# nubot-nudt/RDMNet

Measured on AMD Instinct MI355X. Metric: scan-pairs/sec (whole node), higher is better.
Workload: dtype f32

## Files before the change

include/rdmnet_hip.h:

```cpp
#ifndef RDMNET_HIP_H_
#define RDMNET_HIP_H_

#include <stddef.h>
#include <stdint.h>

#ifdef __cplusplus
extern "C" {
#endif

#define RDM_ABI_VERSION 2

int rdm_abi_version(void);
size_t rdm_abi_struct_size(int which);
const char* rdm_last_error(void);

int rdm_rehash_schedule(int64_t max_elems, int64_t* at_host, int64_t* buckets_host, int cap);

size_t rdm_grid_subsample_workspace_bytes(int64_t n_points, int batch);
int rdm_grid_subsample(const float* points, int64_t n_points, const int64_t* lengths, int batch,
                       float voxel_size, float* out_points, int64_t* out_lengths, void* ws,
                       size_t ws_bytes, void* stream);
int rdm_grid_subsample_form(const float* points, int64_t n_points, const int64_t* lengths, int batch, float voxel_size,
                            float* out_points, int64_t* out_lengths, void* ws, size_t ws_bytes, void* stream, int form);

// ... 95 lines not shown
                                  double* out);
size_t rdm_pose_graph_consistency_workspace_bytes(int64_t n_graphs, const int64_t* graph_node_offsets_host,
                                                  const int64_t* graph_edge_offsets_host, const int64_t* edges_host,
                                                  const int64_t* graph_pair_offsets_host, const int64_t* pairs_host);
int rdm_pose_graph_consistency(int64_t n_graphs, const int64_t* graph_node_offsets_host, const int64_t* graph_edge_offsets_host,
                               const double* nodes, const int64_t* edges_host, const double* transforms, const double* informations,
                               const double* weights, const int64_t* graph_pair_offsets_host, const int64_t* pairs_host,
                               const double* pair_transforms, const double* pair_informations, double* covariances_out,
                               double* cross_out, double* residual_cov_out, double* d2_out, uint8_t* pair_status_out,
                               double* report_host, void* ws, size_t ws_bytes, void* stream);
int rdm_pose_graph_pair_covariances_host(int64_t n_nodes, int64_t n_edges, const int64_t* edges_host, const double* diag,
                                         const double* off, int64_t n_pairs, const int64_t* pairs_host, double* out);
int rdm_pose_graph_pair_terms_host(const double* source_pose, const double* target_pose, const double* transform,
                                   const double* information, const double* cov_ss, const double* cov_tt, const double* cov_st,
                                   double* out);
int rdm_dbg_pose_graph_marginals_ticks(long long* device_ticks);

size_t rdm_gemm_workspace_bytes(int64_t m, int64_t n, int batches);
int rdm_gemm(const float* a, int64_t lda, int64_t stride_a, const float* b, int64_t ldb,
             int64_t stride_b, int trans_b, float* c, int64_t ldc, int64_t stride_c, int64_t m,
             int64_t n, int64_t k, int batches, const float* bias, const float* rowdiv, int act,
             void* ws, size_t ws_bytes, void* stream);
int rdm_gemm_last_plan(int* out4_host);

int rdm_kpconv_gather(const float* q_points, int64_t m, const float* s_points, int64_t n_s,
                      const float* s_feats, int64_t c, int64_t ldf, const uint8_t* s_positive,
                      const int64_t* idx, int64_t h, int64_t ldi, const int32_t* width,
                      const float* kernel_points, float sigma, float* wf, int64_t ldw, float* nn,
                      void* stream);
int rdm_kpconv_fused_enabled(void);
int rdm_kpconv_fused_supported(int64_t c_in, int64_t c_out);
int64_t rdm_kpconv_fused_partial_rows(int64_t m, int64_t c_in);
size_t rdm_kpconv_packed_floats(int64_t c_in, int64_t c_out);
int rdm_kpconv_pack_weights(const float* w_host, int64_t c_in, int64_t c_out, float* packed_host);
int rdm_kpconv_fused(const float* q_points, int64_t m, const float* s_points, int64_t n_s, const float* s_feats,
                     int64_t c, int64_t ldf, const uint8_t* s_positive, const int64_t* idx, int64_t h, int64_t ldi,
                     const int32_t* width, const float* kernel_points, float sigma, const float* w_packed,
                     const float* bias, int64_t c_out, float* out, int64_t ldo, double* gn_partial,
                     const float* order_records, void* stream);
int rdm_kpconv_fused_form(const float* q_points, int64_t m, const float* s_points, int64_t n_s, const float* s_feats,
                          int64_t c, int64_t ldf, const uint8_t* s_positive, const int64_t* idx, int64_t h, int64_t ldi,
                          const int32_t* width, const float* kernel_points, float sigma, const float* w_packed,
                          const float* bias, int64_t c_out, float* out, int64_t ldo, double* gn_partial,
                          const float* order_records, int form, void* stream);
size_t rdm_kpconv_fused_workspace_bytes(int64_t m, int64_t c_in, int64_t c_out);
int rdm_kpconv_fused_group_norm(const float* q_points, int64_t m, const float* s_points, int64_t n_s,
// ... 418 lines not shown
```

rdmnet_amd/_lib.py:

```python
import ctypes
import os

_HERE = os.path.dirname(os.path.abspath(__file__))
LIB_PATH = os.environ.get('RDM_LIB_PATH') or os.path.join(_HERE, 'librdmnet_hip.so')

c_void = ctypes.c_void_p
c_i64 = ctypes.c_int64
c_int = ctypes.c_int
c_f32 = ctypes.c_float
c_size = ctypes.c_size_t

ABI_VERSION = 2


class FineMatchingOptions(ctypes.Structure):
    _fields_ = [('topk', ctypes.c_int32), ('mutual', ctypes.c_int32), ('use_dustbin', ctypes.c_int32),
                ('use_global_score', ctypes.c_int32), ('confidence_threshold', ctypes.c_float),
                ('correspondence_limit', ctypes.c_int32)]

    @classmethod
    def of(cls, topk=1, mutual=False, use_dustbin=True, confidence_threshold=0.0, use_global_score=False,
           correspondence_limit=None):
        return cls(int(topk), int(bool(mutual)), int(bool(use_dustbin)), int(bool(use_global_score)), float(confidence_threshold),
                   0 if correspondence_limit is None else int(correspondence_limit))
# ... 36 lines not shown
               'bad_indices')

SIGNATURES = {
    'rdm_abi_version': (c_int, []),
    'rdm_abi_struct_size': (c_size, [c_int]),
    'rdm_last_error': (ctypes.c_char_p, []),
    'rdm_rehash_schedule': (c_int, [c_i64, c_void, c_void, c_int]),
    'rdm_grid_subsample_workspace_bytes': (c_size, [c_i64, c_int]),
    'rdm_grid_subsample': (c_int, [c_void, c_i64, c_void, c_int, c_f32, c_void, c_void, c_void, c_size,
                                   c_void]),
    'rdm_grid_subsample_form': (c_int, [c_void, c_i64, c_void, c_int, c_f32, c_void, c_void, c_void, c_size,
                                        c_void, c_int]),
    'rdm_radius_neighbors_workspace_bytes': (c_size, [c_i64, c_i64, c_int]),
    'rdm_radius_neighbors': (c_int, [c_void, c_i64, c_void, c_i64, c_void, c_void, c_int, c_f32, c_int,
                                     c_void, c_void, c_void, c_void, c_void, c_size, c_void]),
    'rdm_radius_grid_workspace_bytes': (c_size, [c_i64]),
    'rdm_radius_grid_build': (c_int, [c_void, c_i64, c_void, c_int, c_f32, c_void, c_size, c_void]),
    'rdm_radius_grid_query': (c_int, [c_void, c_size, c_i64, c_void, c_i64, c_void, c_int, c_f32, c_int, c_void, c_void,
                                      c_void, c_void, c_void, c_size, c_void]),
    'rdm_gemm_workspace_bytes': (c_size, [c_i64, c_i64, c_int]),
    'rdm_gemm': (c_int, [c_void, c_i64, c_i64, c_void, c_i64, c_i64, c_int, c_void, c_i64, c_i64, c_i64, c_i64,
                         c_i64, c_int, c_void, c_void, c_int, c_void, c_size, c_void]),
    'rdm_gemm_last_plan': (c_int, [c_void]),
    'rdm_kpconv_gather': (c_int, [c_void, c_i64, c_void, c_i64, c_void, c_i64, c_i64, c_void, c_void, c_i64,
                                  c_i64, c_void, c_void, c_f32, c_void, c_i64, c_void, c_void]),
    'rdm_kpconv_gather_ordered': (c_int, [c_void, c_i64, c_void, c_i64, c_void, c_i64, c_i64, c_void, c_void, c_i64,
                                          c_i64, c_void, c_void, c_f32, c_void, c_i64, c_void, c_void, c_void]),
    'rdm_kpconv_gather_form': (c_int, [c_void, c_i64, c_void, c_i64, c_void, c_i64, c_i64, c_void, c_void, c_i64,
                                       c_i64, c_void, c_void, c_f32, c_void, c_i64, c_void, c_void, c_int, c_void]),
    'rdm_kpconv_fused_enabled': (c_int, []),
    'rdm_kpconv_fused_supported': (c_int, [c_i64, c_i64]),
    'rdm_kpconv_fused_partial_rows': (c_i64, [c_i64, c_i64]),
    'rdm_kpconv_packed_floats': (c_size, [c_i64, c_i64]),
    'rdm_kpconv_pack_weights': (c_int, [c_void, c_i64, c_i64, c_void]),
    'rdm_kpconv_fused': (c_int, [c_void, c_i64, c_void, c_i64, c_void, c_i64, c_i64, c_void, c_void, c_i64, c_i64, c_void, c_void,
                                 c_f32, c_void, c_void, c_i64, c_void, c_i64, c_void, c_void, c_void]),
    'rdm_kpconv_fused_form': (c_int, [c_void, c_i64, c_void, c_i64, c_void, c_i64, c_i64, c_void, c_void, c_i64, c_i64, c_void, c_void,
                                      c_f32, c_void, c_void, c_i64, c_void, c_i64, c_void, c_void, c_int, c_void]),
    'rdm_kpconv_fused_workspace_bytes': (c_size, [c_i64, c_i64, c_i64]),
    'rdm_kpconv_fused_group_norm': (c_int, [c_void, c_i64, c_void, c_i64, c_void, c_i64, c_i64, c_void, c_void, c_i64, c_i64, c_void,
                                            c_void, c_f32, c_void, c_void, c_i64, c_int, c_void, c_void, c_f32, c_int, c_void, c_i64,
                                            c_void, c_i64, c_void, c_size, c_void, c_void]),
    'rdm_voxel_downsample_workspace_bytes': (c_size, [c_i64]),
    'rdm_voxel_downsample': (c_int, [c_void, c_i64, c_i64, c_int, ctypes.c_double, c_void, c_i64, c_void, c_void, c_void,
                                     c_size, c_void]),
    'rdm_ransac_workspace_bytes': (c_size, [c_int]),
# ... 270 lines not shown
```

rdmnet_amd/csrc/gemm.hip:

```cpp
#include "../../include/rdmnet_hip.h"
#include <cmath>
#include <cstdlib>

#include "common.h"
#include "internal.h"
#include "lockstep.h"

namespace {

using namespace rdm;

typedef float f32x16 __attribute__((ext_vector_type(16)));
typedef float f32x4_t __attribute__((ext_vector_type(4)));

struct GemmArgs {
  const float* A = nullptr;
  const float* B = nullptr;
  float* C = nullptr;
  const float* bias = nullptr;
  const float* rowdiv = nullptr;
  int M = 0, N = 0, K = 0;
  int lda = 0, ldb = 0, ldc = 0;
  long long sa = 0, sb = 0, sc = 0;
  int act = 0;
  int splits = 1;
  float* part = nullptr;
  double* stats = nullptr;
  const float* A2 = nullptr;
  const int64_t* aidx = nullptr;
  int lda2 = 0, ldi = 0, c1 = 0, n_coarse = 0;
  const int64_t* bidx = nullptr;
  int n_b = 0;
  const float* seed = nullptr;
  const int64_t* sidx = nullptr;
  int ld_seed = 0, ldsi = 0, n_seed = 0;
  int xcd_tiles = 0;
#ifdef RDM_GEMM_TIMING
  unsigned long long* clk = nullptr;
#endif
};
#ifdef RDM_GEMM_TIMING
#define GEMM_STAMP(k) do { if (blockIdx.x == 0 && blockIdx.y == 0 && blockIdx.z == 0 && threadIdx.x == 0) g.clk[k] = __builtin_amdgcn_s_memtime(); } while (0)
#else
#define GEMM_STAMP(k) do { } while (0)
#endif

__device__ __forceinline__ float apply_act(float v, int act) {
  if (act == 1) return v > 0.f ? v : 0.f;
  if (act == 2) return v > 0.f ? v : 0.1f * v;
  return v;
}

template <int BM, int BN, int WM, int WN, int BK, bool TRANS_B, int PF, bool CAT = false, bool SEED = false>
__device__ __forceinline__ void gemm_kernel_body(const dim3 blockIdx, const dim3 gridDim, GemmArgs g) {
  (void)blockIdx; (void)gridDim;
  constexpr int TM = BM / WM, TN = BN / WN, FM = TM / 32, FN = TN / 32;
  static_assert(WM * WN == 4 && TM % 32 == 0 && TN % 32 == 0, "bad tile");
  static_assert(!SEED || (!CAT && !TRANS_B), "seeded accumulators: plain operands only");
  constexpr int LDA_S = BM + 1, LDB_S = TRANS_B ? BN + 1 : BN + 4;
  constexpr int CR = BM < 64 ? BM : 64;
  constexpr int LDC_S = BN + 4;
  constexpr int TPR = BN / 4;
  constexpr int RPI = 256 / TPR;
  constexpr int kBytesAB = (2 * BK * LDA_S + 2 * BK * LDB_S) * 4, kBytesC = CR * LDC_S * 4, kBytesStat = RPI * BN * 2 * 8;
  constexpr int kBytes = kBytesAB > kBytesC ? (kBytesAB > kBytesStat ? kBytesAB : kBytesStat) : (kBytesC > kBytesStat ? kBytesC : kBytesStat);
  static_assert((2 * BK * LDA_S * 4) % 16 == 0 && CR % RPI == 0, "tile layout");
  __shared__ __attribute__((aligned(16))) char smem[kBytes];
  float (*As)[BK][LDA_S] = reinterpret_cast<float (*)[BK][LDA_S]>(smem);
  float (*Bs)[BK][LDB_S] = reinterpret_cast<float (*)[BK][LDB_S]>(smem + 2 * BK * LDA_S * 4);
  float (*Cs)[LDC_S] = reinterpret_cast<float (*)[LDC_S]>(smem);
  double (*stat_red)[1][2] = reinterpret_cast<double (*)[1][2]>(smem);

  const int tid = threadIdx.x, lane = tid & 63, wave = tid >> 6;
  const int wm = wave / WN, wn = wave % WN;
  int tile_x = blockIdx.x, tile_y = blockIdx.y;
  if (g.xcd_tiles) {
    const int nblk = gridDim.x * gridDim.y, lin = blockIdx.y * gridDim.x + blockIdx.x;
    const int q = nblk / 8, rr = nblk % 8, xcd = lin % 8, within = lin / 8;
    const int logical = (xcd < rr ? xcd * (q + 1) : rr * (q + 1) + (xcd - rr) * q) + within;
    tile_x = logical % gridDim.x;
    tile_y = logical / gridDim.x;
  }
  const int m0 = tile_y * BM, n0 = tile_x * BN;
  GEMM_STAMP(0);
  const int batch = blockIdx.z / g.splits, split = blockIdx.z % g.splits;
  const float* A = g.A + batch * g.sa;
  const float* B = g.B + batch * g.sb;

  const int ktiles = (g.K + BK - 1) / BK;
  const int per = (ktiles + g.splits - 1) / g.splits;
  const int kt0 = split * per, kt1 = min(ktiles, kt0 + per);

  constexpr int A_N4 = BM * BK / 4;
  constexpr int A_V = (A_N4 + 255) / 256;
// ... 197 lines not shown
          for (int r = 0; r < 16; ++r) {
            const float v = g.seed[max(seed_row[i][r], 0ll) * g.ld_seed + min(col, g.N - 1)];
            acc[i][j][r] = (seed_row[i][r] >= 0 && col < g.N) ? v : 0.f;
          }
        }
    }
    store_tiles(ra0, rb0, 0, kt0);
  }
  lds_barrier();
  GEMM_STAMP(1);
  if (kt0 < kt1) {
    read_half(af_lo, bf_lo, 0, 0);
    if constexpr (PF == 1) {
      for (int kt = kt0; kt < kt1; ++kt) step(ra0, rb0, ra0, rb0, kt, (kt - kt0) & 1);
    } else {
      for (int kt = kt0; kt < kt1; kt += 2) {
        step(ra0, rb0, ra1, rb1, kt, 0);
        if (kt + 1 < kt1) step(ra1, rb1, ra0, rb0, kt + 1, 1);
      }
    }
  }

  GEMM_STAMP(2);
  const bool stats = g.stats != nullptr && !partial;
  const bool has_rd = !partial && g.rowdiv != nullptr;
  const int act = g.act;
  float* C = partial ? g.part + static_cast<long long>(blockIdx.z) * g.M * g.N : g.C + batch * g.sc;
  const int ldc = partial ? g.N : g.ldc;
  const bool vec_ok = (ldc & 3) == 0 && (reinterpret_cast<uintptr_t>(C) & 15) == 0;
  double cs[4] = {0.0, 0.0, 0.0, 0.0}, css[4] = {0.0, 0.0, 0.0, 0.0};
#pragma unroll
  for (int pass = 0; pass < BM / CR; ++pass) {
#pragma unroll
    for (int i = 0; i < FM; ++i) {
      const int rbase = wm * TM + i * 32 - pass * CR;
      if (rbase < 0 || rbase >= CR) continue;
#pragma unroll
      for (int j = 0; j < FN; ++j)
#pragma unroll
        for (int r = 0; r < 16; ++r) Cs[rbase + (r & 3) + 8 * (r >> 2) + 4 * lk][wn * TN + j * 32 + li] = acc[i][j][r];
    }
    lds_barrier();
    GEMM_STAMP(4);
#pragma unroll
    for (int it = 0; it < CR / RPI; ++it) {
      const int lrow = it * RPI + rsub;
      const int row = m0 + pass * CR + lrow;
      if (row < g.M && gcol < g.N) {
        const float4 t = *reinterpret_cast<const float4*>(&Cs[lrow][c4]);
        float v[4] = {t.x, t.y, t.z, t.w};
        if (has_rd) {
          const float rd = rdv[pass * (CR / RPI) + it];
#pragma unroll
          for (int e = 0; e < 4; ++e) v[e] = v[e] / rd;
        }
        if (!partial) {
#pragma unroll
          for (int e = 0; e < 4; ++e) {
            const float u = v[e] + bv[e];
            const float neg = act == 2 ? 0.1f * u : 0.f;
            v[e] = (act != 0 && !(u > 0.f)) ? neg : u;
          }
        }
        float* dst = C + static_cast<long long>(row) * ldc + gcol;
        if (vec_ok && gcol + 3 < g.N) {
          *reinterpret_cast<float4*>(dst) = make_float4(v[0], v[1], v[2], v[3]);
        } else {
#pragma unroll
          for (int e = 0; e < 4; ++e)
            if (gcol + e < g.N) dst[e] = v[e];
        }
        if (stats) {
#pragma unroll
          for (int e = 0; e < 4; ++e) {
            cs[e] += v[e];
            css[e] += static_cast<double>(v[e]) * v[e];
          }
        }
      }
    }
    GEMM_STAMP(5);
    lds_barrier();
  }
  if (stats) {
#pragma unroll
    for (int e = 0; e < 4; ++e) {
      stat_red[rsub * BN + c4 + e][0][0] = cs[e];
      stat_red[rsub * BN + c4 + e][0][1] = css[e];
    }
    lds_barrier();
    for (int cl = tid; cl < BN; cl += 256) {
      const int col = n0 + cl;
      if (col >= g.N) continue;
      double a = 0.0, b = 0.0;
#pragma unroll
      for (int w = 0; w < RPI; ++w) {
        a += stat_red[w * BN + cl][0][0];
        b += stat_red[w * BN + cl][0][1];
      }
      g.stats[(static_cast<long long>(tile_y) * 2 + 0) * g.N + col] = a;
      g.stats[(static_cast<long long>(tile_y) * 2 + 1) * g.N + col] = b;
    }
  }
  GEMM_STAMP(3);
}

__device__ __forceinline__ void gemm_small_body(const dim3 blockIdx, const GemmArgs& g, float (*red)[32][33]) {
  const int tid = threadIdx.x, lane = tid & 63, wave = tid >> 6;
  const int li = lane & 31, lk = lane >> 5;
  const int m0 = blockIdx.y * 32, n0 = blockIdx.x * 32;
  const int kq = g.K / 4;
  const int kbeg = wave * kq;
  const int row = min(m0 + li, g.M - 1);
  const int col = n0 + li;
  const bool col_ok = col < g.ldb;
  const float* arow = g.A + static_cast<long long>(row) * g.lda;
  f32x16 acc;
#pragma unroll
  for (int r = 0; r < 16; ++r) acc[r] = 0.f;
  for (int c = 0; c < kq; c += 32) {
    float a[16], b[16];
    const int kb = kbeg + c + lk * 16;
#pragma unroll
    for (int q = 0; q < 4; ++q) {
      float4 v = make_float4(0.f, 0.f, 0.f, 0.f);
      if (c + lk * 16 + 4 * q < kq) v = *reinterpret_cast<const float4*>(arow + kb + 4 * q);
      a[4 * q] = v.x; a[4 * q + 1] = v.y; a[4 * q + 2] = v.z; a[4 * q + 3] = v.w;
// ... 360 lines not shown
  constexpr int kMinWaves = BM * BN <= 64 * 64 ? 4 : 1;
  static const int pad_env = [] { const char* v = ::rdm::dev_knob("RDM_GEMM_LDS_PAD"); return v ? atoi(v) : -1; }();
  const unsigned pad = pad_env >= 0 ? static_cast<unsigned>(pad_env) : g_lds_pad;
  if constexpr (BM == 64 && BN == 64 && BK == 32 && PF == 2) {
    if (g.aidx && g.bidx) {
      ::rdm::launch<gemm_kernel_body<BM, BN, WM, WN, BK, true, PF, true>, 256, kMinWaves>(grid, pad, st, g);
      return;
    }
    if (g.aidx) {
      ::rdm::launch<gemm_kernel_body<BM, BN, WM, WN, BK, false, PF, true>, 256, kMinWaves>(grid, pad, st, g);
      return;
    }
    if (g.seed) {
      ::rdm::launch<gemm_kernel_body<BM, BN, WM, WN, BK, false, PF, false, true>, 256, kMinWaves>(grid, pad, st, g);
      return;
    }
  }
  if (trans_b)
    ::rdm::launch<gemm_kernel_body<BM, BN, WM, WN, BK, true, PF>, 256, kMinWaves>(grid, pad, st, g);
  else
    ::rdm::launch<gemm_kernel_body<BM, BN, WM, WN, BK, false, PF>, 256, kMinWaves>(grid, pad, st, g);
}

}

void rdm::gemm_set_lds_pad(unsigned bytes) { g_lds_pad = bytes; }

extern "C" size_t rdm_gemm_workspace_bytes(int64_t m, int64_t n, int batches) {
  const size_t by_shape = static_cast<size_t>(m) * static_cast<size_t>(n) * 16;
  const size_t by_tiles = static_cast<size_t>(1024) * 128 * 128;
  return align_up(std::min(by_shape, by_tiles) * sizeof(float) * static_cast<size_t>(batches > 0 ? batches : 1));
}

namespace {

thread_local int g_last_plan[4] = {0, 0, 0, 0};

enum Tile { T128, T64, T128x32 };

struct GemmPlan {
  bool small = false;
  Tile tile = T64;
  int bm = 64, bn = 64, bk = 32;
  int splits = 1;
  int exp_tile = 0;
  int xcd_tiles = 0;
};

bool small_kernel_ok(long long m, long long n, long long k) {
  return m <= 1536 && k % 16 == 0 && k >= 64 && k <= 1024 && m * n <= 1536 * 512;
}

void set_tile_shape(GemmPlan& p, long long k, bool gathered) {
  p.bm = p.tile == T64 ? 64 : 128;
  p.bn = p.tile == T128 ? 128 : (p.tile == T64 ? 64 : 32);
  p.bk = p.tile == T128 ? 16 : ((p.tile == T64 ? (k >= 48 || gathered) : k >= 32) ? 32 : 16);
}

GemmPlan plan_tiled(const GemmArgs& g, int batches, size_t ws_cap, long long model_cus = 256) {
  const long long m = g.M, n = g.N, k = g.K;
  struct Cand { Tile tile; int bm, bn; double fixed_us, lat_k64_us, mfma_k64_us; int resident; double alpha; };
  static const Cand cands[3] = {{T128, 128, 128, 4.0, 2.6, 3.4, 3, 0.0}, {T64, 64, 64, 1.5, 2.2, 0.86, 4, 0.2},
                                {T128x32, 128, 32, 3.0, 1.3, 0.86, 3, 0.0}};
  static const int split_set[8] = {1, 2, 3, 4, 6, 8, 12, 16};
  GemmPlan p;
  double best = 1e30;
  for (const Cand& c : cands) {
    if (g.aidx && c.tile != T64) continue;
    if (c.tile == T128x32 && n > 64) continue;
    if (c.tile != T128x32 && n <= 32) continue;
    if (c.tile == T128 && n < 128) continue;
    const long long tiles = ceil_div<long long>(m, c.bm) * ceil_div<long long>(n, c.bn) * batches;
    const int max_s = k >= 256 ? static_cast<int>(std::min<long long>(16, k / 128)) : 1;
    for (int sp : split_set) {
      if (sp > max_s) break;
      if (sp > 1 && static_cast<size_t>(m) * n * sp * batches * sizeof(float) > ws_cap) break;
      const long long blocks = tiles * sp;
      const double k_per = static_cast<double>(k) / sp / 64.0;
      const long long per_round = model_cus * c.resident;
      const long long full = blocks / per_round, rem = blocks % per_round;
      auto per_k64 = [&](double r) { return std::max(c.lat_k64_us * (1.0 + c.alpha * (r - 1.0)), c.mfma_k64_us * r); };
      double t = full * (c.fixed_us + k_per * per_k64(c.resident));
      if (rem) t += c.fixed_us + k_per * per_k64(static_cast<double>(ceil_div<long long>(rem, model_cus)));
      if (sp > 1) t += 3.0 + static_cast<double>(m) * n * sp * 8.0 / 1.5e6;
      if (t < best) {
        best = t;
        p.tile = c.tile;
        p.splits = sp;
      }
    }
  }
  if (g.aidx && g.bidx) p.splits = 1;
  set_tile_shape(p, k, g.aidx != nullptr);
  return p;
}

GemmPlan plan_gemm(const GemmArgs& g, int batches, bool trans_b, size_t ws_cap) {
  if (batches == 1 && !trans_b && !g.rowdiv && !g.stats && !g.aidx && small_kernel_ok(g.M, g.N, g.K)) {
    GemmPlan p;
    p.small = true;
    p.bm = p.bn = 32; p.bk = g.K / 4; p.splits = 4;
    return p;
  }
  return plan_tiled(g, batches, ws_cap);
}

#ifdef RDM_DEV_KNOBS

bool lab_tune_skips_small() {
  const char* tune = ::rdm::dev_knob("RDM_GEMM_TUNE");
  return tune && tune[0] != '0';
}

void lab_overrides(GemmPlan& p, const GemmArgs& g, int batches, size_t ws_cap) {
  const long long m = g.M, n = g.N, k = g.K;
  static const long long model_cus = [] {
    const char* v = ::rdm::dev_knob("RDM_GEMM_CUS");
    const long long n = v ? atoll(v) : 256;
    return n >= 8 && n <= 256 ? n : 256ll;
  }();
  if (p.small && !lab_tune_skips_small()) return;
  if (p.small || model_cus != 256) p = plan_tiled(g, batches, ws_cap, model_cus);
  int force_splits = 0;
  if (const char* tune = ::rdm::dev_knob("RDM_GEMM_TUNE")) {
    int t = 0, sp = 0;
    if (sscanf(tune, "%d,%d", &t, &sp) >= 1) {
      if (t == 1) p.tile = T128;
      else if (t == 2) p.tile = T64;
      else if (t == 3) p.tile = T128x32;
      else if (t >= 4 && t <= 7) p.exp_tile = t;
      force_splits = sp;
      if (t >= 1 && t <= 7 && sp == 0) p.splits = 1;
    }
  }
  static const int big_min_m = [] { const char* v = ::rdm::dev_knob("RDM_GEMM_BIG"); return v ? atoi(v) : 0; }();
  static const int big_tile = [] { const char* v = ::rdm::dev_knob("RDM_GEMM_BIG"); const char* c = v ? strchr(v, ',') : nullptr; return c ? atoi(c + 1) : 6; }();
  static const bool big_split = ::rdm::dev_knob("RDM_GEMM_BIG_SPLIT") != nullptr;
  if (big_min_m > 0 && big_tile >= 4 && big_tile <= 7 && p.exp_tile == 0 && m >= big_min_m && n >= 128 && (p.splits == 1 || big_split) && force_splits == 0 && batches == 1)
    p.exp_tile = big_tile;
  static const bool xcd_env = ::rdm::dev_knob("RDM_GEMM_XCD") != nullptr;
  p.xcd_tiles = (xcd_env && ceil_div<long long>(n, 64) > 1 && ceil_div<long long>(m, 64) * ceil_div<long long>(n, 64) >= 64) ? 1 : 0;
  if (g.aidx) {
    p.tile = T64;
    p.exp_tile = 0;
    if (g.bidx) p.splits = 1, force_splits = 0;
  }
  if (force_splits > 0)
    p.splits = (force_splits > 1 && static_cast<size_t>(m) * n * force_splits * batches * sizeof(float) <= ws_cap) ? force_splits : 1;
  set_tile_shape(p, k, g.aidx != nullptr);
  static const bool bk16 = ::rdm::dev_knob("RDM_GEMM_BK16") != nullptr;
  if (bk16 && p.tile == T64 && !g.aidx) p.bk = 16;
  if (p.exp_tile) {
    p.bm = p.exp_tile == 5 ? 64 : (p.exp_tile == 7 ? 256 : 128);
    p.bn = (p.exp_tile == 5 || p.exp_tile == 6) ? 128 : 64;
    p.bk = 32;
  }
}
#endif

int launch_plan(const GemmPlan& p, GemmArgs g, int batches, bool trans_b, void* ws, int* stat_blocks, hipStream_t st) {
  const long long m = g.M, n = g.N;
  g_last_plan[0] = p.bm; g_last_plan[1] = p.bn; g_last_plan[2] = p.bk; g_last_plan[3] = p.splits;
  if (g.seed && (p.small || p.exp_tile || p.tile != T64 || p.bk != 32 || p.splits != 1 || batches != 1 || trans_b || g.aidx)) {
    set_error("gemm: seeded accumulators exist for the un-split 64 x 64 x 32 tile only");
    return RDM_ERR_ARG;
  }
  if (p.small) {
    if (stat_blocks) *stat_blocks = 0;
    RDM_DUP_LOOP("gemmsmall")
    ::rdm::launch<gemm_small_entry, 256>(dim3(ceil_div<long long>(n, 32), ceil_div<long long>(m, 32)), 0, st, g);
    return launch_status("gemm_small_kernel");
  }
  g.xcd_tiles = p.xcd_tiles;
  if (p.splits > 1) {
    g.splits = p.splits;
    g.part = static_cast<float*>(ws);
  }
  double* reduce_stats = nullptr;
  if (g.splits > 1) {
    if (batches == 1 && g.N % 4 == 0) reduce_stats = g.stats;
    g.stats = nullptr;
  }
  if (stat_blocks)
    *stat_blocks = g.stats ? static_cast<int>(ceil_div<long long>(m, p.bm))
                           : (reduce_stats ? static_cast<int>(ceil_div<long long>(m, stat_rows_per_block(n))) : 0);
  RDM_DUP_LOOP("gemm") {
#ifdef RDM_DEV_KNOBS
  if (p.exp_tile == 4) launch<128, 64, 2, 2, 32, 2>(g, batches, trans_b, st);
  else if (p.exp_tile == 5) launch<64, 128, 2, 2, 32, 2>(g, batches, trans_b, st);
  else if (p.exp_tile == 6) launch<128, 128, 2, 2, 32, 2>(g, batches, trans_b, st);
  else if (p.exp_tile == 7) launch<256, 64, 4, 1, 32, 2>(g, batches, trans_b, st);
  else
#endif
  switch (p.tile) {
    case T128: launch<128, 128, 2, 2, 16>(g, batches, trans_b, st); break;
    case T64:
      if (p.bk == 32) launch<64, 64, 2, 2, 32, 2>(g, batches, trans_b, st);
      else launch<64, 64, 2, 2, 16>(g, batches, trans_b, st);
      break;
    case T128x32:
      if (p.bk == 32) launch<128, 32, 4, 1, 32, 2>(g, batches, trans_b, st);
      else launch<128, 32, 4, 1, 16>(g, batches, trans_b, st);
      break;
  }
  }
  if (int e = launch_status("gemm_kernel")) return e;
  if (g.splits > 1 && reduce_stats) {
    RDM_DUP_LOOP("splitk")
    ::rdm::launch<splitk_reduce_stats_kernel_body, 256>(dim3(ceil_div<long long>(m, stat_rows_per_block(n)), ceil_div<long long>(n, 256)), 0, st, g, reduce_stats);
    return launch_status("splitk_reduce_stats_kernel");
  }
  if (g.splits > 1) {
    const long long total = static_cast<long long>(batches) * m * n;
    const int blocks = static_cast<int>(std::min<long long>(ceil_div<long long>(total, 256), 2048));
    ::rdm::launch<splitk_reduce_kernel_body, 256>(dim3(blocks), 0, st, g, batches);
    return launch_status("splitk_reduce_kernel");
  }
  return RDM_OK;
}

int gemm_dispatch(const GemmArgs& g, int batches, bool trans_b, void* ws, size_t ws_bytes, int* stat_blocks, hipStream_t st) {
  const size_t ws_cap = ws ? ws_bytes : 0;
  GemmPlan p = plan_gemm(g, batches, trans_b, ws_cap);
#ifdef RDM_DEV_KNOBS
  lab_overrides(p, g, batches, ws_cap);
#endif
  return launch_plan(p, g, batches, trans_b, ws, stat_blocks, st);
}

}

int rdm::gemm_with_stats(const float* a, int64_t lda, const float* b, int64_t ldb, float* c, int64_t ldc, int64_t m,
                         int64_t n, int64_t k, const float* bias, const float* rowdiv, void* ws, size_t ws_bytes,
                         double* gn_partial, int* gn_blocks, void* stream) {
  GemmArgs g;
  g.A = a; g.B = b; g.C = c; g.bias = bias; g.rowdiv = rowdiv;
  g.M = static_cast<int>(m); g.N = static_cast<int>(n); g.K = static_cast<int>(k);
  g.lda = static_cast<int>(lda); g.ldb = static_cast<int>(ldb); g.ldc = static_cast<int>(ldc);
  g.stats = gn_partial;
  return gemm_dispatch(g, 1, false, ws, ws_bytes, gn_blocks, static_cast<hipStream_t>(stream));
}

int rdm::gemm_concat_with_stats(const float* coarse, int64_t ld1, int64_t c1, int64_t n_coarse, const int64_t* idx, int64_t ldi,
                                const float* skip, int64_t ld2, int64_t c2, const float* b, int64_t ldb, float* c, int64_t ldc,
                                int64_t m, int64_t n, int64_t n_need, const float* bias, int act, float* pbuf, size_t pbuf_floats,
                                void* ws, size_t ws_bytes, double* gn_partial, int* gn_blocks, void* stream) {
  if (c1 % 32 != 0 || c2 % 4 != 0 || c2 < 4 || ld1 % 4 != 0 || ld2 % 4 != 0 || ldb % 4 != 0 || m <= 0 ||
      ((reinterpret_cast<uintptr_t>(coarse) | reinterpret_cast<uintptr_t>(skip) | reinterpret_cast<uintptr_t>(b)) & 15) != 0)
    return 1;
  GemmArgs g;
  g.A = coarse; g.B = b; g.C = c; g.bias = bias;
  g.M = static_cast<int>(m); g.N = static_cast<int>(n); g.K = static_cast<int>(c1 + c2);
  g.lda = static_cast<int>(ld1); g.ldb = static_cast<int>(ldb); g.ldc = static_cast<int>(ldc);
  g.act = act; g.stats = gn_partial;
  g.A2 = skip; g.aidx = idx; g.lda2 = static_cast<int>(ld2); g.ldi = static_cast<int>(ldi); g.c1 = static_cast<int>(c1);
  g.n_coarse = static_cast<int>(n_coarse);
  hipStream_t st = static_cast<hipStream_t>(stream);
  const size_t ws_cap = ws ? ws_bytes : 0;
  GemmPlan p = plan_gemm(g, 1, false, ws_cap);
#ifdef RDM_DEV_KNOBS
  lab_overrides(p, g, 1, ws_cap);
#endif
  if (p.splits == 1) n = n_need;
  g.N = static_cast<int>(n);
  const int64_t ldp = (n + 3) / 4 * 4;
  const bool seeded = p.splits == 1 && p.tile == T64 && p.bk == 32 && p.exp_tile == 0 && n_coarse > 0 && n_coarse < m &&
                      pbuf && static_cast<size_t>(n_coarse) * ldp <= pbuf_floats && (reinterpret_cast<uintptr_t>(pbuf) & 15) == 0;
  if (!seeded) return launch_plan(p, g, 1, false, ws, gn_blocks, st);
  GemmArgs gp;
  gp.A = coarse; gp.B = b; gp.C = pbuf;
  gp.M = static_cast<int>(n_coarse); gp.N = static_cast<int>(n); gp.K = static_cast<int>(c1);
  gp.lda = static_cast<int>(ld1); gp.ldb = static_cast<int>(ldb); gp.ldc = static_cast<int>(ldp);
  const GemmPlan pp = plan_tiled(gp, 1, 0);
  if (int e = launch_plan(pp, gp, 1, false, nullptr, nullptr, st)) return e;
  GemmArgs gs;
  gs.A = skip; gs.B = b + c1 * ldb; gs.C = c; gs.bias = bias;
  gs.M = static_cast<int>(m); gs.N = static_cast<int>(n); gs.K = static_cast<int>(c2);
  gs.lda = static_cast<int>(ld2); gs.ldb = static_cast<int>(ldb); gs.ldc = static_cast<int>(ldc);
  gs.act = act; gs.stats = gn_partial;
  gs.seed = pbuf; gs.ld_seed = static_cast<int>(ldp); gs.sidx = idx; gs.ldsi = static_cast<int>(ldi); gs.n_seed = static_cast<int>(n_coarse);
  GemmPlan ps;
  ps.tile = T64; ps.splits = 1;
  set_tile_shape(ps, c2, true);
  return launch_plan(ps, gs, 1, false, nullptr, gn_blocks, st);
}

int rdm::gemm_pair(const float* a0, int64_t lda0, const float* b0, int64_t ldb0, float* c0, int64_t ldc0, int64_t m0, int64_t n0,
                   int64_t k0, const float* bias0, const float* a1, int64_t lda1, const float* b1, int64_t ldb1, float* c1,
                   int64_t ldc1, int64_t m1, int64_t n1, int64_t k1, const float* bias1, void* ws, size_t ws_bytes, void* stream) {
  bool small = m0 > 0 && m1 > 0 && small_kernel_ok(m0, n0, k0) && small_kernel_ok(m1, n1, k1) && lda0 % 4 == 0 && lda1 % 4 == 0 &&
               ldb0 % 4 == 0 && ldb1 % 4 == 0 && ((reinterpret_cast<uintptr_t>(a0) | reinterpret_cast<uintptr_t>(a1)) & 15) == 0;
#ifdef RDM_DEV_KNOBS
  small = small && !lab_tune_skips_small();
#endif
  if (small) {
    GemmArgs g[2];
    const float* A[2] = {a0, a1}; const float* B[2] = {b0, b1}; float* C[2] = {c0, c1}; const float* bias[2] = {bias0, bias1};
    const int64_t M[2] = {m0, m1}, N[2] = {n0, n1}, K[2] = {k0, k1}, LA[2] = {lda0, lda1}, LB[2] = {ldb0, ldb1}, LC[2] = {ldc0, ldc1};
    for (int i = 0; i < 2; ++i) {
      g[i].A = A[i]; g[i].B = B[i]; g[i].C = C[i]; g[i].bias = bias[i];
      g[i].M = static_cast<int>(M[i]); g[i].N = static_cast<int>(N[i]); g[i].K = static_cast<int>(K[i]);
      g[i].lda = static_cast<int>(LA[i]); g[i].ldb = static_cast<int>(LB[i]); g[i].ldc = static_cast<int>(LC[i]);
    }
    const long long gx = ceil_div<long long>(std::max(n0, n1), 32), gy = ceil_div<long long>(std::max(m0, m1), 32);
    ::rdm::launch<gemm_small_pair_entry, 256>(dim3(gx, gy, 2), 0, static_cast<hipStream_t>(stream), g[0], g[1]);
    return launch_status("gemm_small_pair_kernel");
  }
  if (m0 > 0)
    if (int e = rdm_gemm(a0, lda0, 0, b0, ldb0, 0, 0, c0, ldc0, 0, m0, n0, k0, 1, bias0, nullptr, 0, ws, ws_bytes, stream)) return e;
  if (m1 > 0) return rdm_gemm(a1, lda1, 0, b1, ldb1, 0, 0, c1, ldc1, 0, m1, n1, k1, 1, bias1, nullptr, 0, ws, ws_bytes, stream);
  return RDM_OK;
}

extern "C" int rdm_gemm_last_plan(int* out4_host) {
  using namespace rdm;
  RDM_REQUIRE(out4_host, "rdm_gemm_last_plan: null pointer");
  for (int i = 0; i < 4; ++i) out4_host[i] = g_last_plan[i];
  return RDM_OK;
}

extern "C" int rdm_gemm(const float* a, int64_t lda, int64_t stride_a, const float* b, int64_t ldb,
                        int64_t stride_b, int trans_b, float* c, int64_t ldc, int64_t stride_c,
                        int64_t m, int64_t n, int64_t k, int batches, const float* bias,
                        const float* rowdiv, int act, void* ws, size_t ws_bytes, void* stream) {
  using namespace rdm;
  RDM_REQUIRE(a && b && c, "rdm_gemm: null pointer");
  RDM_REQUIRE(m >= 0 && n >= 0 && k >= 0 && batches >= 1, "rdm_gemm: bad sizes");
  if (m == 0 || n == 0) return RDM_OK;
  RDM_REQUIRE(k % 4 == 0 && lda % 4 == 0 && ldb % 4 == 0,
              "rdm_gemm: K (%lld), lda (%lld), ldb (%lld) must be multiples of 4 (pad with zeros)",
              (long long)k, (long long)lda, (long long)ldb);
  RDM_REQUIRE((reinterpret_cast<uintptr_t>(a) & 15) == 0 && (reinterpret_cast<uintptr_t>(b) & 15) == 0,
              "rdm_gemm: A and B must be 16-byte aligned");
  RDM_REQUIRE(act >= 0 && act <= 2, "rdm_gemm: unknown activation %d", act);
  GemmArgs g;
  g.A = a; g.B = b; g.C = c; g.bias = bias; g.rowdiv = rowdiv;
  g.M = static_cast<int>(m); g.N = static_cast<int>(n); g.K = static_cast<int>(k);
  g.lda = static_cast<int>(lda); g.ldb = static_cast<int>(ldb); g.ldc = static_cast<int>(ldc);
  g.sa = stride_a; g.sb = stride_b; g.sc = stride_c;
  g.act = act;
  return gemm_dispatch(g, batches, trans_b != 0, ws, ws_bytes, nullptr, static_cast<hipStream_t>(stream));
}
// ... 182 lines not shown
```

Measured before the change: 617.7.

## Add row-streaming GEMM kernel that keeps B resident and walks several row tiles

Adds a GEMM variant for tall, small-K problems (K up to 128, M at least 2048): each workgroup loads the whole B panel into LDS once, then loops over up to four 64-row tiles of A. It prefetches the next A tile into registers while the current tile runs its MFMAs. The epilogue is split out into a shared helper. The goal is to cut repeated B loads and the launch and prologue cost of many tiny workgroups. The trade-offs are fewer workgroups, which can under-fill the GPU, and higher LDS use per block. The path is on by default through the planner for eligible shapes.

```diff
diff --git a/include/rdmnet_hip.h b/include/rdmnet_hip.h
--- a/include/rdmnet_hip.h
+++ b/include/rdmnet_hip.h
@@ -141,6 +141,8 @@
              int64_t n, int64_t k, int batches, const float* bias, const float* rowdiv, int act,
              void* ws, size_t ws_bytes, void* stream);
 int rdm_gemm_last_plan(int* out4_host);
+int rdm_gemm_set_row_streaming(int on);
+int rdm_gemm_last_row_tiles(void);
 
 int rdm_kpconv_gather(const float* q_points, int64_t m, const float* s_points, int64_t n_s,
                       const float* s_feats, int64_t c, int64_t ldf, const uint8_t* s_positive,
diff --git a/rdmnet_amd/_lib.py b/rdmnet_amd/_lib.py
--- a/rdmnet_amd/_lib.py
+++ b/rdmnet_amd/_lib.py
@@ -82,6 +82,8 @@
     'rdm_gemm': (c_int, [c_void, c_i64, c_i64, c_void, c_i64, c_i64, c_int, c_void, c_i64, c_i64, c_i64, c_i64,
                          c_i64, c_int, c_void, c_void, c_int, c_void, c_size, c_void]),
     'rdm_gemm_last_plan': (c_int, [c_void]),
+    'rdm_gemm_set_row_streaming': (c_int, [c_int]),
+    'rdm_gemm_last_row_tiles': (c_int, []),
     'rdm_kpconv_gather': (c_int, [c_void, c_i64, c_void, c_i64, c_void, c_i64, c_i64, c_void, c_void, c_i64,
                                   c_i64, c_void, c_void, c_f32, c_void, c_i64, c_void, c_void]),
     'rdm_kpconv_gather_ordered': (c_int, [c_void, c_i64, c_void, c_i64, c_void, c_i64, c_i64, c_void, c_void, c_i64,
diff --git a/rdmnet_amd/csrc/gemm.hip b/rdmnet_amd/csrc/gemm.hip
--- a/rdmnet_amd/csrc/gemm.hip
+++ b/rdmnet_amd/csrc/gemm.hip
@@ -1,4 +1,6 @@
 #include "../../include/rdmnet_hip.h"
+#include <algorithm>
+#include <atomic>
 #include <cmath>
 #include <cstdlib>
 
@@ -34,6 +36,7 @@
   const float* seed = nullptr;
   const int64_t* sidx = nullptr;
   int ld_seed = 0, ldsi = 0, n_seed = 0;
+  int row_tiles = 0;
   int xcd_tiles = 0;
 #ifdef RDM_GEMM_TIMING
   unsigned long long* clk = nullptr;
@@ -49,6 +52,105 @@
   if (act == 1) return v > 0.f ? v : 0.f;
   if (act == 2) return v > 0.f ? v : 0.1f * v;
   return v;
+}
+
+template <int BM, int BN, int WM, int WN>
+__device__ __forceinline__ void gemm_epilogue(const dim3 blockIdx, const GemmArgs& g, char* smem, const f32x16 (&acc)[BM / WM / 32][BN / WN / 32],
+                                              int m0, int n0, int tile_y, int batch, bool partial, const float (&bv)[4],
+                                              const float (&rdv)[BM / (256 / (BN / 4))]) {
+  (void)blockIdx;
+  constexpr int TM = BM / WM, TN = BN / WN, FM = TM / 32, FN = TN / 32;
+  constexpr int CR = BM < 64 ? BM : 64;
+  constexpr int LDC_S = BN + 4;
+  constexpr int TPR = BN / 4;
+  constexpr int RPI = 256 / TPR;
+  float (*Cs)[LDC_S] = reinterpret_cast<float (*)[LDC_S]>(smem);
+  double (*stat_red)[1][2] = reinterpret_cast<double (*)[1][2]>(smem);
+  const int tid = threadIdx.x, lane = tid & 63, wave = tid >> 6;
+  const int wm = wave / WN, wn = wave % WN;
+  const int lk = lane >> 5, li = lane & 31;
+  const int c4 = (tid % TPR) * 4, rsub = tid / TPR;
+  const int gcol = n0 + c4;
+  const bool stats = g.stats != nullptr && !partial;
+  const bool has_rd = !partial && g.rowdiv != nullptr;
+  const int act = g.act;
+  float* C = partial ? g.part + static_cast<long long>(blockIdx.z) * g.M * g.N : g.C + batch * g.sc;
+  const int ldc = partial ? g.N : g.ldc;
+  const bool vec_ok = (ldc & 3) == 0 && (reinterpret_cast<uintptr_t>(C) & 15) == 0;
+  double cs[4] = {0.0, 0.0, 0.0, 0.0}, css[4] = {0.0, 0.0, 0.0, 0.0};
+#pragma unroll
+  for (int pass = 0; pass < BM / CR; ++pass) {
+#pragma unroll
+    for (int i = 0; i < FM; ++i) {
+      const int rbase = wm * TM + i * 32 - pass * CR;
+      if (rbase < 0 || rbase >= CR) continue;
+#pragma unroll
+      for (int j = 0; j < FN; ++j)
+#pragma unroll
+        for (int r = 0; r < 16; ++r) Cs[rbase + (r & 3) + 8 * (r >> 2) + 4 * lk][wn * TN + j * 32 + li] = acc[i][j][r];
+    }
+    lds_barrier();
+    GEMM_STAMP(4);
+#pragma unroll
+    for (int it = 0; it < CR / RPI; ++it) {
+      const int lrow = it * RPI + rsub;
+      const int row = m0 + pass * CR + lrow;
+      if (row < g.M && gcol < g.N) {
+        const float4 t = *reinterpret_cast<const float4*>(&Cs[lrow][c4]);
+        float v[4] = {t.x, t.y, t.z, t.w};
+        if (has_rd) {
+          const float rd = rdv[pass * (CR / RPI) + it];
+#pragma unroll
+          for (int e = 0; e < 4; ++e) v[e] = v[e] / rd;
+        }
+        if (!partial) {
+#pragma unroll
+          for (int e = 0; e < 4; ++e) {
+            const float u = v[e] + bv[e];
+            const float neg = act == 2 ? 0.1f * u : 0.f;
+            v[e] = (act != 0 && !(u > 0.f)) ? neg : u;
+          }
+        }
+        float* dst = C + static_cast<long long>(row) * ldc + gcol;
+        if (vec_ok && gcol + 3 < g.N) {
+          *reinterpret_cast<float4*>(dst) = make_float4(v[0], v[1], v[2], v[3]);
+        } else {
+#pragma unroll
+          for (int e = 0; e < 4; ++e)
+            if (gcol + e < g.N) dst[e] = v[e];
+        }
+        if (stats) {
+#pragma unroll
+          for (int e = 0; e < 4; ++e) {
+            cs[e] += v[e];
+            css[e] += static_cast<double>(v[e]) * v[e];
+          }
+        }
+      }
+    }
+    GEMM_STAMP(5);
+    lds_barrier();
+  }
+  if (stats) {
+#pragma unroll
+    for (int e = 0; e < 4; ++e) {
+      stat_red[rsub * BN + c4 + e][0][0] = cs[e];
+      stat_red[rsub * BN + c4 + e][0][1] = css[e];
+    }
+    lds_barrier();
+    for (int cl = tid; cl < BN; cl += 256) {
+      const int col = n0 + cl;
+      if (col >= g.N) continue;
+      double a = 0.0, b = 0.0;
+#pragma unroll
+      for (int w = 0; w < RPI; ++w) {
+        a += stat_red[w * BN + cl][0][0];
+        b += stat_red[w * BN + cl][0][1];
+      }
+      g.stats[(static_cast<long long>(tile_y) * 2 + 0) * g.N + col] = a;
+      g.stats[(static_cast<long long>(tile_y) * 2 + 1) * g.N + col] = b;
+    }
+  }
 }
 
 template <int BM, int BN, int WM, int WN, int BK, bool TRANS_B, int PF, bool CAT = false, bool SEED = false>
@@ -68,8 +170,6 @@
   __shared__ __attribute__((aligned(16))) char smem[kBytes];
   float (*As)[BK][LDA_S] = reinterpret_cast<float (*)[BK][LDA_S]>(smem);
   float (*Bs)[BK][LDB_S] = reinterpret_cast<float (*)[BK][LDB_S]>(smem + 2 * BK * LDA_S * 4);
-  float (*Cs)[LDC_S] = reinterpret_cast<float (*)[LDC_S]>(smem);
-  double (*stat_red)[1][2] = reinterpret_cast<double (*)[1][2]>(smem);
 
   const int tid = threadIdx.x, lane = tid & 63, wave = tid >> 6;
   const int wm = wave / WN, wn = wave % WN;
@@ -313,87 +413,134 @@
   }
 
   GEMM_STAMP(2);
-  const bool stats = g.stats != nullptr && !partial;
-  const bool has_rd = !partial && g.rowdiv != nullptr;
-  const int act = g.act;
-  float* C = partial ? g.part + static_cast<long long>(blockIdx.z) * g.M * g.N : g.C + batch * g.sc;
-  const int ldc = partial ? g.N : g.ldc;
-  const bool vec_ok = (ldc & 3) == 0 && (reinterpret_cast<uintptr_t>(C) & 15) == 0;
-  double cs[4] = {0.0, 0.0, 0.0, 0.0}, css[4] = {0.0, 0.0, 0.0, 0.0};
-#pragma unroll
-  for (int pass = 0; pass < BM / CR; ++pass) {
-#pragma unroll
-    for (int i = 0; i < FM; ++i) {
-      const int rbase = wm * TM + i * 32 - pass * CR;
-      if (rbase < 0 || rbase >= CR) continue;
-#pragma unroll
-      for (int j = 0; j < FN; ++j)
-#pragma unroll
-        for (int r = 0; r < 16; ++r) Cs[rbase + (r & 3) + 8 * (r >> 2) + 4 * lk][wn * TN + j * 32 + li] = acc[i][j][r];
+  gemm_epilogue<BM, BN, WM, WN>(blockIdx, g, smem, acc, m0, n0, tile_y, batch, partial, bv, rdv);
+  GEMM_STAMP(3);
+}
+
+template <int NH, int KMAX>
+__device__ __forceinline__ void gemm_rows_body(const dim3 blockIdx, const dim3 gridDim, GemmArgs g) {
+  (void)gridDim;
+  constexpr int BN = 64 * NH, LDA_S = 65, LDB_S = BN + 4;
+  constexpr int kBytesB = KMAX * LDB_S * 4, kBytesA = KMAX * LDA_S * 4, kBytesC = 64 * 68 * 4;
+  constexpr int kBytesU = kBytesA > kBytesC ? kBytesA : kBytesC;
+  static_assert(kBytesB % 16 == 0 && KMAX % 16 == 0, "tile layout");
+  __shared__ __attribute__((aligned(16))) char smem[kBytesB + kBytesU];
+  float (*Bs)[LDB_S] = reinterpret_cast<float (*)[LDB_S]>(smem);
+  char* const smem_u = smem + kBytesB;
+  float (*As)[LDA_S] = reinterpret_cast<float (*)[LDA_S]>(smem_u);
+
+  const int tid = threadIdx.x, lane = tid & 63, wave = tid >> 6;
+  const int wm = wave >> 1, wn = wave & 1, lk = lane >> 5, li = lane & 31;
+  const int n0 = blockIdx.x * BN;
+  const int tiles = (g.M + 63) / 64;
+  const int tile0 = blockIdx.y * g.row_tiles, tile1 = min(tiles, tile0 + g.row_tiles);
+  const int K = g.K, KP = (K + 7) & ~7, KC4 = K >> 2;
+
+  constexpr int A_V = KMAX / 16, B_V = KMAX * BN / 1024;
+  int a_row[A_V], a_kc[A_V];
+#pragma unroll
+  for (int i = 0; i < A_V; ++i) {
+    const int idx = tid + i * 256;
+    a_row[i] = idx / KC4;
+    a_kc[i] = (idx - a_row[i] * KC4) * 4;
+  }
+  float4 ra[A_V];
+  auto load_a = [&](int tile) {
+#pragma unroll
+    for (int i = 0; i < A_V; ++i)
+      ra[i] = *reinterpret_cast<const float4*>(g.A + static_cast<long long>(min(tile * 64 + min(a_row[i], 63), g.M - 1)) * g.lda + a_kc[i]);
+  };
+  auto store_a = [&](int tile) {
+#pragma unroll
+    for (int i = 0; i < A_V; ++i) {
+      if (a_row[i] >= 64) continue;
+      const bool ok = tile * 64 + a_row[i] < g.M;
+      As[a_kc[i] + 0][a_row[i]] = ok ? ra[i].x : 0.f;
+      As[a_kc[i] + 1][a_row[i]] = ok ? ra[i].y : 0.f;
+      As[a_kc[i] + 2][a_row[i]] = ok ? ra[i].z : 0.f;
+      As[a_kc[i] + 3][a_row[i]] = ok ? ra[i].w : 0.f;
+    }
+    if (KP > K) As[K + wave][lane] = 0.f;
+  };
+
+  load_a(tile0);
+  {
+    float4 rb[B_V];
+#pragma unroll
+    for (int i = 0; i < B_V; ++i) {
+      const int idx = tid + i * 256;
+      const int k = idx / (BN / 4), n4 = (idx % (BN / 4)) * 4;
+      rb[i] = *reinterpret_cast<const float4*>(g.B + static_cast<long long>(min(k, K - 1)) * g.ldb + min(n0 + n4, g.ldb - 4));
+    }
+#pragma unroll
+    for (int i = 0; i < B_V; ++i) {
+      const int idx = tid + i * 256;
+      const int k = idx / (BN / 4), n4 = (idx % (BN / 4)) * 4;
+      const bool ok = k < K && n0 + n4 < g.ldb;
+      *reinterpret_cast<float4*>(&Bs[k][n4]) = make_float4(ok ? rb[i].x : 0.f, ok ? rb[i].y : 0.f, ok ? rb[i].z : 0.f, ok ? rb[i].w : 0.f);
+    }
+  }
+  const int c4 = (tid % 16) * 4, rsub = tid / 16;
+  float bv[NH][4];
+#pragma unroll
+  for (int h = 0; h < NH; ++h)
+#pragma unroll
+    for (int e = 0; e < 4; ++e) {
+      const int col = n0 + 64 * h + c4 + e;
+      bv[h][e] = (g.bias && col < g.N) ? g.bias[min(col, g.N - 1)] : 0.f;
+    }
+  store_a(tile0);
+  lds_barrier();
+
+  for (int tile = tile0; tile < tile1; ++tile) {
+    const int m0 = tile * 64;
+    load_a(min(tile + 1, tile1 - 1));
+    float rdv[4];
+#pragma unroll
+    for (int q = 0; q < 4; ++q) rdv[q] = g.rowdiv ? g.rowdiv[min(m0 + q * 16 + rsub, g.M - 1)] : 1.f;
+    __builtin_amdgcn_sched_barrier(0);
+
+    f32x16 acc[NH][1][1];
+#pragma unroll
+    for (int h = 0; h < NH; ++h)
+#pragma unroll
+      for (int r = 0; r < 16; ++r) acc[h][0][0][r] = 0.f;
+    float a0[4], b0[4][NH], a1[4], b1[4][NH];
+    auto read8 = [&](float (&a)[4], float (&b)[4][NH], int k0) {
+#pragma unroll
+      for (int s = 0; s < 4; ++s) {
+        a[s] = As[k0 + 2 * s + lk][wm * 32 + li];
+#pragma unroll
+        for (int h = 0; h < NH; ++h) b[s][h] = Bs[k0 + 2 * s + lk][64 * h + wn * 32 + li];
+      }
+    };
+    auto mma8 = [&](const float (&a)[4], const float (&b)[4][NH]) {
+#pragma unroll
+      for (int s = 0; s < 4; ++s)
+#pragma unroll
+        for (int h = 0; h < NH; ++h) acc[h][0][0] = __builtin_amdgcn_mfma_f32_32x32x2f32(a[s], b[s][h], acc[h][0][0], 0, 0, 0);
+    };
+    read8(a0, b0, 0);
+    for (int k0 = 0; k0 < KP; k0 += 16) {
+      read8(a1, b1, min(k0 + 8, KP - 8));
+      mma8(a0, b0);
+      if (k0 + 8 >= KP) break;
+      read8(a0, b0, min(k0 + 16, KP - 8));
+      mma8(a1, b1);
     }
     lds_barrier();
-    GEMM_STAMP(4);
-#pragma unroll
-    for (int it = 0; it < CR / RPI; ++it) {
-      const int lrow = it * RPI + rsub;
-      const int row = m0 + pass * CR + lrow;
-      if (row < g.M && gcol < g.N) {
-        const float4 t = *reinterpret_cast<const float4*>(&Cs[lrow][c4]);
-        float v[4] = {t.x, t.y, t.z, t.w};
-        if (has_rd) {
-          const float rd = rdv[pass * (CR / RPI) + it];
-#pragma unroll
-          for (int e = 0; e < 4; ++e) v[e] = v[e] / rd;
-        }
-        if (!partial) {
-#pragma unroll
-          for (int e = 0; e < 4; ++e) {
-            const float u = v[e] + bv[e];
-            const float neg = act == 2 ? 0.1f * u : 0.f;
-            v[e] = (act != 0 && !(u > 0.f)) ? neg : u;
-          }
-        }
-        float* dst = C + static_cast<long long>(row) * ldc + gcol;
-        if (vec_ok && gcol + 3 < g.N) {
-          *reinterpret_cast<float4*>(dst) = make_float4(v[0], v[1], v[2], v[3]);
-        } else {
-#pragma unroll
-          for (int e = 0; e < 4; ++e)
-            if (gcol + e < g.N) dst[e] = v[e];
-        }
-        if (stats) {
-#pragma unroll
-          for (int e = 0; e < 4; ++e) {
-            cs[e] += v[e];
-            css[e] += static_cast<double>(v[e]) * v[e];
-          }
-        }
-      }
-    }
-    GEMM_STAMP(5);
-    lds_barrier();
-  }
-  if (stats) {
-#pragma unroll
-    for (int e = 0; e < 4; ++e) {
-      stat_red[rsub * BN + c4 + e][0][0] = cs[e];
-      stat_red[rsub * BN + c4 + e][0][1] = css[e];
-    }
-    lds_barrier();
-    for (int cl = tid; cl < BN; cl += 256) {
-      const int col = n0 + cl;
-      if (col >= g.N) continue;
-      double a = 0.0, b = 0.0;
-#pragma unroll
-      for (int w = 0; w < RPI; ++w) {
-        a += stat_red[w * BN + cl][0][0];
-        b += stat_red[w * BN + cl][0][1];
-      }
-      g.stats[(static_cast<long long>(tile_y) * 2 + 0) * g.N + col] = a;
-      g.stats[(static_cast<long long>(tile_y) * 2 + 1) * g.N + col] = b;
-    }
-  }
-  GEMM_STAMP(3);
+
+#pragma unroll
+    for (int h = 0; h < NH; ++h) {
+      if (n0 + 64 * h >= g.N) continue;
+      gemm_epilogue<64, 64, 2, 2>(blockIdx, g, smem_u, acc[h], m0, n0 + 64 * h, tile, 0, false, bv[h], rdv);
+      lds_barrier();
+    }
+    if (tile + 1 < tile1) {
+      store_a(tile + 1);
+      lds_barrier();
+    }
+  }
 }
 
 __device__ __forceinline__ void gemm_small_body(const dim3 blockIdx, const GemmArgs& g, float (*red)[32][33]) {
@@ -800,6 +947,25 @@
     ::rdm::launch<gemm_kernel_body<BM, BN, WM, WN, BK, false, PF>, 256, kMinWaves>(grid, pad, st, g);
 }
 
+template <int NH, int KMAX>
+void launch_rows_nk(const GemmArgs& g, hipStream_t st) {
+  dim3 grid(ceil_div(g.N, 64 * NH), ceil_div(ceil_div(g.M, 64), g.row_tiles), 1);
+  constexpr int kMinWaves = KMAX <= 32 ? 4 : (KMAX <= 64 ? 3 : 2);
+  static const int pad_env = [] { const char* v = ::rdm::dev_knob("RDM_GEMM_LDS_PAD"); return v ? atoi(v) : -1; }();
+  const unsigned pad = pad_env >= 0 ? static_cast<unsigned>(pad_env) : g_lds_pad;
+  ::rdm::launch<gemm_rows_body<NH, KMAX>, 256, kMinWaves>(grid, pad, st, g);
+}
+template <int NH>
+void launch_rows_n(const GemmArgs& g, hipStream_t st) {
+  if (g.K <= 32) launch_rows_nk<NH, 32>(g, st);
+  else if (g.K <= 64) launch_rows_nk<NH, 64>(g, st);
+  else launch_rows_nk<NH, 128>(g, st);
+}
+void launch_rows(const GemmArgs& g, hipStream_t st) {
+  if (g.N > 64 && g.N <= 128) launch_rows_n<2>(g, st);
+  else launch_rows_n<1>(g, st);
+}
+
 }
 
 void rdm::gemm_set_lds_pad(unsigned bytes) { g_lds_pad = bytes; }
@@ -821,12 +987,28 @@
   Tile tile = T64;
   int bm = 64, bn = 64, bk = 32;
   int splits = 1;
+  int rows = 0;
   int exp_tile = 0;
   int xcd_tiles = 0;
 };
 
 bool small_kernel_ok(long long m, long long n, long long k) {
   return m <= 1536 && k % 16 == 0 && k >= 64 && k <= 1024 && m * n <= 1536 * 512;
+}
+
+std::atomic<int> g_row_streaming{1};
+thread_local int g_last_rows = 0;
+
+constexpr int kRowsMaxK = 128, kRowsMinM = 2048, kRowsTargetWgs = 128, kRowsMaxTiles = 4;
+void set_rows(GemmPlan& p, const GemmArgs& g, int batches, bool trans_b, int max_k = kRowsMaxK, int min_m = kRowsMinM, int force_rows = 0) {
+  p.rows = 0;
+  const int mode = g_row_streaming.load(std::memory_order_relaxed);
+  if (mode == 0) return;
+  if (mode == 2) min_m = 1, force_rows = force_rows > 0 ? force_rows : kRowsMaxTiles;
+  if (p.small || p.exp_tile || p.tile != T64 || p.splits != 1 || batches != 1 || trans_b || g.aidx || g.bidx || g.seed) return;
+  if (g.K < 4 || g.K > max_k || g.K % 4 != 0 || g.N < 64 || g.M < min_m) return;
+  const int tiles = ceil_div(g.M, 64);
+  p.rows = force_rows > 0 ? force_rows : std::max(1, std::min(kRowsMaxTiles, tiles / kRowsTargetWgs));
 }
 
 void set_tile_shape(GemmPlan& p, long long k, bool gathered) {
@@ -835,7 +1017,7 @@
   p.bk = p.tile == T128 ? 16 : ((p.tile == T64 ? (k >= 48 || gathered) : k >= 32) ? 32 : 16);
 }
 
-GemmPlan plan_tiled(const GemmArgs& g, int batches, size_t ws_cap, long long model_cus = 256) {
+GemmPlan plan_tiled(const GemmArgs& g, int batches, bool trans_b, size_t ws_cap, long long model_cus = 256) {
   const long long m = g.M, n = g.N, k = g.K;
   struct Cand { Tile tile; int bm, bn; double fixed_us, lat_k64_us, mfma_k64_us; int resident; double alpha; };
   static const Cand cands[3] = {{T128, 128, 128, 4.0, 2.6, 3.4, 3, 0.0}, {T64, 64, 64, 1.5, 2.2, 0.86, 4, 0.2},
@@ -870,6 +1052,7 @@
   }
   if (g.aidx && g.bidx) p.splits = 1;
   set_tile_shape(p, k, g.aidx != nullptr);
+  set_rows(p, g, batches, trans_b);
   return p;
 }
 
@@ -880,7 +1063,7 @@
     p.bm = p.bn = 32; p.bk = g.K / 4; p.splits = 4;
     return p;
   }
-  return plan_tiled(g, batches, ws_cap);
+  return plan_tiled(g, batches, trans_b, ws_cap);
 }
 
 #ifdef RDM_DEV_KNOBS
@@ -890,7 +1073,7 @@
   return tune && tune[0] != '0';
 }
 
-void lab_overrides(GemmPlan& p, const GemmArgs& g, int batches, size_t ws_cap) {
+void lab_overrides(GemmPlan& p, const GemmArgs& g, int batches, bool trans_b, size_t ws_cap) {
   const long long m = g.M, n = g.N, k = g.K;
   static const long long model_cus = [] {
     const char* v = ::rdm::dev_knob("RDM_GEMM_CUS");
@@ -898,7 +1081,7 @@
     return n >= 8 && n <= 256 ? n : 256ll;
   }();
   if (p.small && !lab_tune_skips_small()) return;
-  if (p.small || model_cus != 256) p = plan_tiled(g, batches, ws_cap, model_cus);
+  if (p.small || model_cus != 256) p = plan_tiled(g, batches, trans_b, ws_cap, model_cus);
   int force_splits = 0;
   if (const char* tune = ::rdm::dev_knob("RDM_GEMM_TUNE")) {
     int t = 0, sp = 0;
@@ -933,12 +1116,17 @@
     p.bn = (p.exp_tile == 5 || p.exp_tile == 6) ? 128 : 64;
     p.bk = 32;
   }
+  static const char* rows_env = ::rdm::dev_knob("RDM_GEMM_ROWS");
+  int max_k = kRowsMaxK, min_m = kRowsMinM, force_rows = 0;
+  if (rows_env) sscanf(rows_env, "%d,%d,%d", &max_k, &min_m, &force_rows);
+  set_rows(p, g, batches, trans_b, std::min(max_k, kRowsMaxK), min_m, std::min(force_rows, 64));
 }
 #endif
 
 int launch_plan(const GemmPlan& p, GemmArgs g, int batches, bool trans_b, void* ws, int* stat_blocks, hipStream_t st) {
   const long long m = g.M, n = g.N;
   g_last_plan[0] = p.bm; g_last_plan[1] = p.bn; g_last_plan[2] = p.bk; g_last_plan[3] = p.splits;
+  g_last_rows = p.rows;
   if (g.seed && (p.small || p.exp_tile || p.tile != T64 || p.bk != 32 || p.splits != 1 || batches != 1 || trans_b || g.aidx)) {
     set_error("gemm: seeded accumulators exist for the un-split 64 x 64 x 32 tile only");
     return RDM_ERR_ARG;
@@ -963,6 +1151,10 @@
     *stat_blocks = g.stats ? static_cast<int>(ceil_div<long long>(m, p.bm))
                            : (reduce_stats ? static_cast<int>(ceil_div<long long>(m, stat_rows_per_block(n))) : 0);
   RDM_DUP_LOOP("gemm") {
+  if (p.rows > 0) {
+    g.row_tiles = p.rows;
+    launch_rows(g, st);
+  } else
 #ifdef RDM_DEV_KNOBS
   if (p.exp_tile == 4) launch<128, 64, 2, 2, 32, 2>(g, batches, trans_b, st);
   else if (p.exp_tile == 5) launch<64, 128, 2, 2, 32, 2>(g, batches, trans_b, st);
@@ -1001,7 +1193,7 @@
   const size_t ws_cap = ws ? ws_bytes : 0;
   GemmPlan p = plan_gemm(g, batches, trans_b, ws_cap);
 #ifdef RDM_DEV_KNOBS
-  lab_overrides(p, g, batches, ws_cap);
+  lab_overrides(p, g, batches, trans_b, ws_cap);
 #endif
   return launch_plan(p, g, batches, trans_b, ws, stat_blocks, st);
 }
@@ -1037,7 +1229,7 @@
   const size_t ws_cap = ws ? ws_bytes : 0;
   GemmPlan p = plan_gemm(g, 1, false, ws_cap);
 #ifdef RDM_DEV_KNOBS
-  lab_overrides(p, g, 1, ws_cap);
+  lab_overrides(p, g, 1, false, ws_cap);
 #endif
   if (p.splits == 1) n = n_need;
   g.N = static_cast<int>(n);
@@ -1049,7 +1241,7 @@
   gp.A = coarse; gp.B = b; gp.C = pbuf;
   gp.M = static_cast<int>(n_coarse); gp.N = static_cast<int>(n); gp.K = static_cast<int>(c1);
   gp.lda = static_cast<int>(ld1); gp.ldb = static_cast<int>(ldb); gp.ldc = static_cast<int>(ldp);
-  const GemmPlan pp = plan_tiled(gp, 1, 0);
+  const GemmPlan pp = plan_tiled(gp, 1, false, 0);
   if (int e = launch_plan(pp, gp, 1, false, nullptr, nullptr, st)) return e;
   GemmArgs gs;
   gs.A = skip; gs.B = b + c1 * ldb; gs.C = c; gs.bias = bias;
@@ -1096,6 +1288,14 @@
   for (int i = 0; i < 4; ++i) out4_host[i] = g_last_plan[i];
   return RDM_OK;
 }
+
+extern "C" int rdm_gemm_set_row_streaming(int on) {
+  RDM_REQUIRE(on >= 0 && on <= 2, "rdm_gemm_set_row_streaming: 0 (off), 1 (on) or 2 (on whatever the number of rows)");
+  g_row_streaming.store(on, std::memory_order_relaxed);
+  return rdm::RDM_OK;
+}
+
+extern "C" int rdm_gemm_last_row_tiles(void) { return g_last_rows; }
 
 extern "C" int rdm_gemm(const float* a, int64_t lda, int64_t stride_a, const float* b, int64_t ldb,
                         int64_t stride_b, int trans_b, float* c, int64_t ldc, int64_t stride_c,
```

Result: no change. 614.2, median of 2 (-0.6%).
